# gvtulder/elasticdeform

Measured on AMD Instinct MI355X. Metric: Mvoxels/s fwd+grad, 256^3 fp32 order=3, higher is better.
Workload: dtype f32; 1 GPU; cfg2: 3D 256x256x256 float32, 5x5x5 grid sigma 5, order 3, mode mirror, prefilter on, deform_grid + deform_grid_gradient per step, one volume per GPU; parallelism=1 volume per GPU, no collective

## Files before the change

elasticdeform_amd/csrc/deform_k1z.hip:

```cpp
#include <hip/hip_runtime.h>

#include <cstring>
#include <type_traits>

#include "ed_device.h"
#include "ed_gridfilter.h"
#include "ed_params.h"
#include "ed_tile.h"
#include "ed_workspace.h"
#include "ed_zwalk.h"

namespace ed {
namespace tile {

#ifdef EDHIP_K1_STATS
__device__ unsigned long long g_k1z_stats[8];
#define ZSTAT(K, N) atomicAdd(&g_k1z_stats[K], (unsigned long long)(N))
#else
#define ZSTAT(K, N) do { } while (0)
#endif

namespace {


// ... 2 lines not shown
    kZStaged = 2,
    kZFast = 4,
    kZDma = 8,
    kZXin = 16,
    kZZYin = 32,
    kZUnfit = 64,
    kZGen = 128,
};
struct ZRecU {
    int b0z, b0y, b0x, flags, pitch, ez, ey, ex, goff, plane;
};
typedef int zv8i __attribute__((ext_vector_type(8)));
typedef const __attribute__((address_space(4))) zv8i* crec_p;
__device__ __forceinline__ ZRecU zrec_unpack(const zv8i& v)
{
    ZRecU r;
    r.b0z = v[0];
    r.b0y = v[1];
    r.b0x = v[2];
    r.flags = v[3];
    r.pitch = (v[3] >> 8) & 255;
    r.ez = v[4] & 1023;
    r.ey = (v[4] >> 10) & 1023;
    r.ex = (int)((unsigned)v[4] >> 20);
    r.goff = v[5];
    r.plane = r.ey * r.pitch;
    return r;
}
__device__ __forceinline__ ZRecU zrec_load(crec_p p)
{
    const zv8i v = *p;
    return zrec_unpack(v);
}

__host__ __device__ __forceinline__ int zctl(int parity, int list, int xcd) { return (parity * 2 + list) * 8 + xcd; }

#define ED_RED6(CTRL)                                      \
    "v_min_i32_dpp %0, %0, %0 " CTRL "\n\t"                \
    "v_min_i32_dpp %1, %1, %1 " CTRL "\n\t"                \
    "v_min_i32_dpp %2, %2, %2 " CTRL "\n\t"                \
    "v_max_i32_dpp %3, %3, %3 " CTRL "\n\t"                \
    "v_max_i32_dpp %4, %4, %4 " CTRL "\n\t"                \
    "v_max_i32_dpp %5, %5, %5 " CTRL "\n\t"
__device__ __forceinline__ void zrow_box(int (&lo)[3], int (&hi)[3])
{
    asm volatile("s_nop 1\n\t"
                 ED_RED6("quad_perm:[1,0,3,2] row_mask:0xf bank_mask:0xf")
                 ED_RED6("quad_perm:[2,3,0,1] row_mask:0xf bank_mask:0xf")
                 ED_RED6("row_half_mirror row_mask:0xf bank_mask:0xf")
                 ED_RED6("row_mirror row_mask:0xf bank_mask:0xf")
                 : "+v"(lo[0]), "+v"(lo[1]), "+v"(lo[2]), "+v"(hi[0]), "+v"(hi[1]), "+v"(hi[2]));
}
#undef ED_RED6
__device__ __forceinline__ int zuni(int v) { return __builtin_amdgcn_readfirstlane(v); }
__device__ __forceinline__ void zlds_barrier() { asm volatile("s_waitcnt lgkmcnt(0)\n\ts_barrier" ::: "memory"); }
__device__ __forceinline__ void zdma_barrier() { asm volatile("s_waitcnt vmcnt(0) lgkmcnt(0)\n\ts_barrier" ::: "memory"); }
__device__ __forceinline__ void zglds16(const float* g, float* lds)
{
    __builtin_amdgcn_global_load_lds((const __attribute__((address_space(1))) void*)g,
                                     (__attribute__((address_space(3))) void*)lds, 16, 0, 0);
}
template <bool OUT16>
__device__ __forceinline__ void zstore_out(float* img, long long off, float val, int io16)
{
    if constexpr (OUT16)
        reinterpret_cast<unsigned short*>(img)[off] = (unsigned short)narrow16(val, io16);
    else
        __builtin_nontemporal_store(val, img + off);
}

__device__ __forceinline__ void zaxis_entry(const GridGeom& g, int a, int oi, double* w, int* idx)
{
    const double cp = control_coordinate(g.ncp[a], (int64_t)oi + g.off[a], g.in_len[a]);
    const int64_t start = window_start(cp, 3);
    const bool edge = start < 0 || start + 3 >= g.ncp[a];
    spline_weights(cp, 3, w);
#pragma unroll
    for (int l = 0; l < 4; ++l)
        idx[l] = edge ? mirror_i32((int)start + l, (int)g.ncp[a]) : (int)start + l;
}

constexpr int kGeoBlock = 256;
constexpr int kGeoWaves = kGeoBlock / 64;
__global__ __launch_bounds__(kGeoBlock) void k1z_geo_kernel(const GridGeom g, const HotGeom hg, const ZGeom zg,
                                                          const GridPrefilter gp)
{
    extern __shared__ __attribute__((aligned(16))) char smem[];
    const int tid = threadIdx.x;
    const int lane = tid & 63;
    const int wave = zuni(tid >> 6);
    const int sample = blockIdx.y;
    const int ncpz = (int)g.ncp[0], ncpy = (int)g.ncp[1], ncpx = (int)g.ncp[2];
    const int nyx = ncpy * ncpx;
    const int ngrid = 3 * ncpz * nyx;
    double* sG = reinterpret_cast<double*>(smem);
    double* sR = sG + ngrid;
    AxTab* sAx = reinterpret_cast<AxTab*>(sR + 64 * ncpz * 3);
    double* sMax = reinterpret_cast<double*>(sAx + 16);
    AxTab* sZ = reinterpret_cast<AxTab*>(sMax + 3 * kGeoWaves);
    int* sCls = reinterpret_cast<int*>(sZ + 4 * hg.tiles[0]);
    int* sBox = sCls + hg.tiles[0];
    int* sCnt = sBox + 64 * hg.tiles[0];
    if ((int)blockIdx.x >= hg.tiles[1] * hg.tiles[2]) {
        const long long nfill = (long long)(gridDim.x - hg.tiles[1] * hg.tiles[2]) * kGeoBlock;
        const long long me = (long long)(blockIdx.x - hg.tiles[1] * hg.tiles[2]) * kGeoBlock + tid;
        const long long n16 = zg.zero_bytes >> 4;
        int4* p16 = reinterpret_cast<int4*>(zg.zero_ptr);
        for (long long i = me; i < n16; i += nfill)
            p16[i] = make_int4(0, 0, 0, 0);
        if (me < (zg.zero_bytes & 15))
            zg.zero_ptr[(n16 << 4) + me] = 0;
        return;
    }
    const int ty = blockIdx.x / hg.tiles[2], tx = blockIdx.x - ty * hg.tiles[2];
    if (ED_DBG(hg.dbg, 1 << 23))
        return;
#ifdef EDHIP_EXPERIMENTS
#define ZTICK(K) do { if (hg.dbgbuf && tid == 0) hg.dbgbuf[(size_t)(blockIdx.x + blockIdx.y * gridDim.x) * 16 + (K)] = __builtin_readcyclecounter(); } while (0)
#else
#define ZTICK(K) do { } while (0)
#endif
    ZTICK(0);

    if (gp.total > 0 && !ED_DBG(hg.dbg, 1 << 28)) {
        grid_prefilter_in_lds<kGeoBlock>(gp, sG, tid);
        if (blockIdx.x == 0 && sample == 0)
            for (int e = tid; e < gp.total; e += kGeoBlock)
                store_cast(gp.out + (int64_t)e * gp.elem_size, gp.dtype, sG[e]);
    } else {
        const char* disp = g.disp + (int64_t)sample * zg.disp_bstride;
        for (int e = tid; e < ngrid; e += kGeoBlock) {
            const int h = e / (ncpz * nyx), r = e - h * (ncpz * nyx);
            const int j0 = r / nyx, j = r - j0 * nyx;
            const int j1 = j / ncpx, j2 = j - j1 * ncpx;
            sG[e] = load_as_double(disp + g.disp_stride[0] * h + g.disp_stride[1] * j0 + g.disp_stride[2] * j1 +
                                       g.disp_stride[3] * j2, g.disp_dtype);
        }
        __syncthreads();
    }
    ZTICK(1);
    if (blockIdx.x == 0 && sample == 0 && tid == 0 && zg.hint) {
        if (zg.hint_host)
            __hip_atomic_store(zg.hint_host, ((unsigned long long)(unsigned)zg.hint[1] << 32) | (unsigned)zg.hint[0],
                               __ATOMIC_RELAXED, __HIP_MEMORY_SCOPE_SYSTEM);
        zg.hint[0] = 0;
        zg.hint[1] = (int)zg.hint_seq;
    }
    for (int h = 0; h < 3 && !ED_DBG(hg.dbg, 1 << 29); ++h) {
        double m = 0.0;
        for (int e = tid; e < ncpz * nyx; e += kGeoBlock)
            m = fmax(m, fabs(sG[h * ncpz * nyx + e]));
        for (int sh = 32; sh >= 1; sh >>= 1)
            m = fmax(m, __shfl_xor(m, sh));
        if (lane == 0)
            sMax[h * kGeoWaves + wave] = m;
    }
    ZTICK(2);
    if (tid < 16 && !ED_DBG(hg.dbg, 1 << 30)) {
        const int a = tid < 8 ? 1 : 2;
        const int oi = min((tid < 8 ? ty : tx) * kT + (tid & 7), hg.out_len[a] - 1);
        AxTab t;
        zaxis_entry(g, a, oi, t.w, t.idx);
        sAx[tid] = t;
    }
    for (int e = tid; e < 4 * hg.tiles[0] && !zg.tables_only && !ED_DBG(hg.dbg, 1 << 26); e += kGeoBlock) {
        const int tz = e >> 2, nz = min(kT, hg.out_len[0] - tz * kT);
        AxTab t;
        zaxis_entry(g, 0, tz * kT + ((e & 3) * (nz - 1)) / 3, t.w, t.idx);
        sZ[e] = t;
    }
    if (blockIdx.x == 0 && sample == 0 && hg.nstep) {
        for (long long ss = tid; ss < hg.nsteps; ss += kGeoBlock) {
            long long vol_off = 0, img_off = 0, r = ss;
            for (int l = 0; l < hg.nstep; ++l) {
                const long long q = r / hg.step_len[l];
                const long long c = r - q * hg.step_len[l];
                vol_off += hg.vol_step[l] * c;
                img_off += hg.img_step[l] * c;
                r = q;
            }
            zg.steps[2 * ss] = vol_off;
            zg.steps[2 * ss + 1] = img_off;
        }
    }
    if (blockIdx.x == 0 && sample == 0 && tid == 0) {
        ZGen* zn = reinterpret_cast<ZGen*>(zg.zgen);
        for (int h = 0; h < 3; ++h) {
            zn->in_len[h] = hg.in_len[h];
            zn->out_len[h] = hg.out_len[h];
            zn->off[h] = hg.off[h];
            zn->period[h] = hg.period[h];
            zn->inv_period[h] = hg.inv_period[h];
            zn->offd[h] = (double)hg.off[h];
        }
        for (int k = 0; k < 12; ++k)
            zn->aff[k] = hg.affine[k];
        zn->mode = hg.mode;
        zn->cval = hg.cval;
        zn->hint = hg.hint;
    }
    if (blockIdx.x == 0 && sample == 0) {
        AxTab* zt = const_cast<AxTab*>(zg.zt);
        for (int oz = tid; oz < hg.out_len[0]; oz += kGeoBlock) {
            AxTab t;
            zaxis_entry(g, 0, oz, t.w, t.idx);
#pragma unroll
            for (int l = 0; l < 4; ++l)
                t.idx[l] *= 32;
            zt[oz] = t;
        }
    }
    __syncthreads();
    ZTICK(3);
    double slack[3];
#pragma unroll
    for (int h = 0; h < 3; ++h) {
        double m = 0.0;
        for (int w = 0; w < kGeoWaves; ++w)
            m = fmax(m, sMax[h * kGeoWaves + w]);
        const double sl = zg.slack_scale * m;
        slack[h] = sl >= 0.02 ? (sl <= 0.75 ? sl : 0.75) : 0.02;
    }
    ZTICK(4);
    if (!ED_DBG(hg.dbg, 1 << 25)) {
        const int col = tid & 63;
        const AxTab ay = sAx[col >> 3];
        const AxTab ax = sAx[8 + (col & 7)];
        int rowoff[4];
#pragma unroll
        for (int ly = 0; ly < 4; ++ly)
            rowoff[ly] = ay.idx[ly] * ncpx;
        for (int r = tid >> 6; r < ncpz * 3; r += kGeoWaves) {
            const int kz = r / 3, h = r - kz * 3;
            const double* gp0 = sG + (h * ncpz + kz) * nyx;
            double acc = 0.0;
#pragma unroll
            for (int ly = 0; ly < 4; ++ly) {
                const double* row = gp0 + rowoff[ly];
                double t = ax.w[0] * row[ax.idx[0]];
#pragma unroll
                for (int lx = 1; lx < 4; ++lx)
                    t = fma(ax.w[lx], row[ax.idx[lx]], t);
                acc = fma(ay.w[ly], t, acc);
            }
            sR[col * (ncpz * 3) + r] = acc;
        }
        __syncthreads();
        double* rg = const_cast<double*>(zg.r) + (int64_t)sample * zg.r_bstride;
        const int rowlen = 8 * 4 * ncpz;
        for (int e = tid; e < 8 * rowlen; e += kGeoBlock) {
            const int py = e / rowlen, j = e - py * rowlen;
            const int px = j / (4 * ncpz), jj = j - px * (4 * ncpz);
            const int kz = jj >> 2, h = jj & 3;
            const int oy = ty * kT + py, ox = tx * kT + px;
            if (oy < hg.out_len[1] && ox < hg.out_len[2])
                rg[((int64_t)oy * hg.out_len[2] + ox) * (4 * ncpz) + jj] = h < 3 ? sR[(py * 8 + px) * (ncpz * 3) + kz * 3 + h] : 0.0;
        }
    }
    if (zg.tables_only)
        return;
    __syncthreads();
    ZTICK(5);
    const int order = zg.order;
    const int H = order / 2, NT = order + 1, kPadX = NT & 1;
    const int ny = min(kT, hg.out_len[1] - ty * kT), nx = min(kT, hg.out_len[2] - tx * kT);
    const int py = (((lane >> 2) & 3) * (ny - 1)) / 3, px = ((lane & 3) * (nx - 1)) / 3;
    const double* rc = sR + (py * 8 + px) * (ncpz * 3);
    for (int tz = wave; tz < hg.tiles[0] && !ED_DBG(hg.dbg, 1 << 24); tz += kGeoWaves) {
        const int nz = min(kT, hg.out_len[0] - tz * kT);
        const int pz = ((lane >> 4) * (nz - 1)) / 3;
        const int o[3] = {tz * kT + pz, ty * kT + py, tx * kT + px};
        const AxTab& ze = sZ[tz * 4 + (lane >> 4)];
        double d[3];
#pragma unroll
        for (int h = 0; h < 3; ++h) {
            d[h] = ze.w[0] * rc[ze.idx[0] * 3 + h];
#pragma unroll
            for (int l = 1; l < 4; ++l)
                d[h] = fma(ze.w[l], rc[ze.idx[l] * 3 + h], d[h]);
        }
        double c[3];
        int lo[3], hi[3];
#pragma unroll
        for (int h = 0; h < 3; ++h) {
            if (hg.has_affine)
                c[h] = fma(hg.affine[h * 4 + 2], (double)o[2],
                           fma(hg.affine[h * 4 + 0], (double)o[0],
                               fma(hg.affine[h * 4 + 1], (double)o[1], hg.affine[h * 4 + 3] + (double)hg.off[h]))) + d[h];
            else
                c[h] = (double)(o[h] + hg.off[h]) + d[h];
            const double cr = (order & 1) ? c[h] : c[h] + 0.5;
            lo[h] = (int)floor(cr - slack[h]);
            hi[h] = (int)floor(cr + slack[h]);
        }
        bool out_of_fast = false;
#pragma unroll
        for (int h = 0; h < 3; ++h)
            out_of_fast = out_of_fast || lo[h] < ((order & 1) ? 0 : 1) || hi[h] > hg.in_len[h] - 2;
        const bool fast = nz == kT && ny == kT && nx == kT && !__any(out_of_fast);
        zrow_box(lo, hi);
        int* dst = sBox + (tz * 8 + (lane >> 4)) * 8;
        if ((lane & 15) == 0) {
#pragma unroll
            for (int h = 0; h < 3; ++h) {
                dst[h] = lo[h];
                dst[4 + h] = hi[h];
            }
        }
        if (lane == 0)
            dst[3] = fast ? 1 : 0;
        if (!fast) {
            bool cst = false;
#pragma unroll
            for (int h = 0; h < 3; ++h) {
                double m = c[h];
                if (!(m >= 0.0 && m <= (double)(hg.in_len[h] - 1)))
                    m = map_coordinate_fast(m, hg.in_len[h], hg.mode, hg.period[h], hg.inv_period[h]);
                cst = cst || !(m > -1.0);
                const double mr = (order & 1) ? m : m + 0.5;
                lo[h] = (int)floor(mr - slack[h]);
                hi[h] = (int)floor(mr + slack[h]);
            }
            if (cst) {
#pragma unroll
                for (int h = 0; h < 3; ++h) {
                    lo[h] = 0x7fffffff;
                    hi[h] = (int)0x80000000;
                }
            }
            zrow_box(lo, hi);
            if ((lane & 15) == 0) {
#pragma unroll
                for (int h = 0; h < 3; ++h) {
                    dst[32 + h] = lo[h];
                    dst[36 + h] = hi[h];
                }
            }
        }
    }
    __syncthreads();
    ZTICK(6);
    for (int tz = tid; tz < hg.tiles[0] && !ED_DBG(hg.dbg, 1 << 27); tz += kGeoBlock) {
        const int tile_id = sample * hg.ntiles + (tz * hg.tiles[1] + ty) * hg.tiles[2] + tx;
        int cls = 0;
        bool hint0 = false, half_fit[2] = {false, false};
#pragma unroll 1
        for (int part = 0; part < 3; ++part) {
            const int* sb = sBox + tz * 64;
            const bool fast = sb[3] != 0;
            const int r0 = part == 2 ? 2 : 0, r1 = part == 1 ? 2 : 3;
            int blo[3], bhi[3];
            bool any = true;
#pragma unroll
            for (int h = 0; h < 3; ++h) {
                int rlo = 0x7fffffff, rhi = (int)0x80000000, lo = 0x7fffffff, hi = (int)0x80000000;
                for (int r = r0; r <= r1; ++r) {
                    rlo = min(rlo, sb[r * 8 + h]);
                    rhi = max(rhi, sb[r * 8 + 4 + h]);
                    lo = min(lo, sb[(fast ? 0 : 32) + r * 8 + h]);
                    hi = max(hi, sb[(fast ? 0 : 32) + r * 8 + 4 + h]);
                }
                if (!fast) {
                    any = any && hi >= lo;
                    const int lowfold = hg.mode == EDHIP_MODE_REFLECT ? -1 : 0;
                    if (rlo < ((order & 1) ? 0 : 1) && rhi >= lowfold)
                        lo = min(lo, lowfold);
                    if (rhi > hg.in_len[h] - 2 && rlo <= hg.in_len[h] - 1)
                        hi = max(hi, hg.in_len[h] - 1);
                }
                blo[h] = lo - H;
                bhi[h] = hi - H + order + (h == 2 ? kPadX : 0);
            }
            if (!any) {
                blo[0] = blo[1] = blo[2] = 0;
                bhi[0] = bhi[1] = bhi[2] = -1;
            }
            any = bhi[0] >= blo[0] && bhi[1] >= blo[1] && bhi[2] >= blo[2];
            unsigned ext[3];
#pragma unroll
            for (int h = 0; h < 3; ++h)
                ext[h] = (unsigned)bhi[h] - (unsigned)blo[h] + 1u;
            const int pitch = ext[2] <= 16u ? 16 : (ext[2] <= 24u ? 24 : (ext[2] <= 32u ? 32 : (ext[2] <= 48u ? 48 : 0)));
            const bool sane = any && ext[0] < 1024u && ext[1] < 1024u;
            const int nrows = sane ? (int)(ext[0] * ext[1]) : 0;
            const bool fits = sane && pitch > 0 && nrows * pitch <= hg.box_cap;
            const bool dma = fits && blo[2] >= 0 && blo[2] + pitch + 1 <= hg.in_len[2];
            const bool xin = fits && blo[2] >= 0 && blo[2] + (int)ext[2] <= hg.in_len[2];
            const bool zyin = fits && blo[0] >= 0 && blo[0] + (int)ext[0] <= hg.in_len[0] && blo[1] >= 0 &&
                              blo[1] + (int)ext[1] <= hg.in_len[1];
            const bool fastA = part == 0 && fast && fits && dma && zyin;
            const int flags = (any ? kZAny : 0) | (fits ? kZStaged : 0) | (fastA ? kZFast : kZGen) | (dma ? kZDma : 0) |
                              (xin ? kZXin : 0) | (zyin ? kZZYin : 0) | (any && !fits ? kZUnfit : 0);
            const int4 w0 = make_int4(blo[0], blo[1], blo[2], flags | (pitch << 8));
            const int4 w1 = make_int4(sane ? (int)(ext[0] | (ext[1] << 10) | (ext[2] << 20)) : 0,
                                      (dma && zyin) ? blo[0] * hg.vol_sz + blo[1] * hg.vol_sy + blo[2] : 0, 0, 0);
            if (part == 0) {
                hint0 = any && !(sane && pitch > 0 && nrows * pitch <= hg.small_cap);
                cls = (flags & kZUnfit) ? 3 : ((flags & kZFast) ? 1 : 2);
                int4* dst = reinterpret_cast<int4*>(zg.recs + (size_t)tile_id * 8);
                dst[0] = w0;
                dst[1] = w1;
                if (hg.boxes) {
                    int* bx = hg.boxes + (size_t)tile_id * 8;
#pragma unroll
                    for (int h = 0; h < 3; ++h) {
                        bx[h] = blo[h];
                        bx[3 + h] = bhi[h] - ((h == 2 && any) ? kPadX : 0);
                    }
                }
                if (cls != 3)
                    break;
            } else {
                half_fit[part - 1] = fits || !any;
                int4* dst = reinterpret_cast<int4*>(zg.recs_half + ((size_t)tile_id * 2 + (part - 1)) * 8);
                dst[0] = w0;
                dst[1] = w1;
            }
        }
        const bool split = cls == 3 && half_fit[0] && half_fit[1];
        ZSTAT(cls == 3 ? (split ? 6 : 5) : (cls == 1 ? 3 : 4), 1);
        sCls[tz] = cls | (split ? 4 : 0) | (hint0 ? 8 : 0);
    }
    __syncthreads();
    ZTICK(7);
    {
        const int zstrips = (hg.tiles[0] + zg.strip_tiles - 1) / zg.strip_tiles;
        if (tid < 4)
            sCnt[tid] = 0;
        __syncthreads();
        int slotG = -1, slotF = -1, sidv = 0;
        if (tid < zstrips) {
            int info = 0;
            bool g = false, f = false;
            for (int k = 0; k < zg.strip_tiles && tid * zg.strip_tiles + k < hg.tiles[0]; ++k) {
                const int c = sCls[tid * zg.strip_tiles + k];
                info |= c << (4 * k);
                g = g || (c & 3) == 2 || (c & 7) == 7;
                f = f || (c & 7) == 3;
            }
            const size_t sid = (size_t)sample * zg.nstrips + ((size_t)tid * hg.tiles[1] + ty) * hg.tiles[2] + tx;
            sidv = (int)sid;
            zg.sinfo[sid] = info;
            zg.missed[sid] = f ? 2 : 0;
            if (g)
                slotG = atomicAdd(&sCnt[0], 1);
            if (f)
                slotF = atomicAdd(&sCnt[1], 1);
        }
        __syncthreads();
        const int xcd = (tx + ty + sample) & 7;
        if (tid == 0) {
            sCnt[2] = sCnt[0] ? atomicAdd(&zg.ctl[zctl(zg.parity, 0, xcd)], sCnt[0]) : 0;
            sCnt[3] = sCnt[1] ? atomicAdd(&zg.ctl[zctl(zg.parity, 1, xcd)], sCnt[1]) : 0;
        }
        if (blockIdx.x == 0 && sample == 0 && tid < 16)
            zg.ctl[zctl(1 - zg.parity, tid >> 3, tid & 7)] = 0;
        __syncthreads();
        if (slotG >= 0)
            zg.list_g[(size_t)(sCnt[2] + slotG) * 8 + xcd] = sidv;
        if (slotF >= 0)
            zg.list_f[(size_t)(sCnt[3] + slotF) * 8 + xcd] = sidv;
    }
    ZTICK(8);
#undef ZTICK
}


struct ZVox {
    int addr[2];
    float frac[2][3];
    int flg;
};
struct ZStrip {
    int tz0, ty, tx, ntile, sample, id;
};
__device__ __forceinline__ bool k1z_strip(int total_strips, int nstrips, int tiles_z, int tiles_y, int tiles_x, int strip_tiles, int deal,
                                          ZStrip& sp, int b)
{
    const int x = b & 7, j = b >> 3;
    const int r = j / deal;
    int s = (r * 8 + ((x + r) & 7)) * deal + (j - r * deal);
    if (s >= total_strips)
        return false;
    sp.id = s;
    sp.sample = s / nstrips;
    s -= sp.sample * nstrips;
    sp.tx = s % tiles_x;
    s /= tiles_x;
    sp.ty = s % tiles_y;
    sp.tz0 = (s / tiles_y) * strip_tiles;
    sp.ntile = min(strip_tiles, tiles_z - sp.tz0);
    return true;
}
inline unsigned k1z_grid(int total_strips, int deal)
{
    const int chunks = (total_strips + deal - 1) / deal;
    return (unsigned)(((chunks + 7) / 8) * 8 * deal);
}

template <int ORDER, int PITCH>
__device__ __forceinline__ float k1z_gather(const float* bp, int plane, int pitch_rt, const float* w0, const float* w1, const float* w2)
{
    constexpr int NT = ORDER + 1;
    constexpr int NTX = NT + (NT & 1);
    float a0 = 0.f;
#pragma unroll
    for (int l0 = 0; l0 < NT; ++l0) {
        const float* pp = bp + l0 * plane;
        float a1 = 0.f;
#pragma unroll
        for (int l1 = 0; l1 < NT; ++l1) {
            const float* rp = pp + l1 * (PITCH ? PITCH : pitch_rt);
            float a2 = 0.f;
#pragma unroll
            for (int l2 = 0; l2 < NTX; l2 += 2) {
                const float2 pr = *reinterpret_cast<const float2*>(rp + l2);
                ED_NO_DS_MERGE();
                a2 = fmaf(w2[l2], pr.x, a2);
                a2 = fmaf(w2[l2 + 1], pr.y, a2);
            }
            a1 = fmaf(w1[l1], a2, a1);
        }
        a0 = fmaf(w0[l0], a1, a0);
    }
    return a0;
}
template <int ORDER>
__device__ __forceinline__ float k1z_voxel(const char* smem, int addr, const float (&frac)[3], int pitch, int plane)
{
    constexpr int NT = ORDER + 1;
    constexpr int NTX = NT + (NT & 1);
    float f0 = frac[0], f1 = frac[1], f2 = frac[2];
    asm volatile("" : "+v"(f0), "+v"(f1), "+v"(f2));
    float w0[NT], w1[NT], w2[NTX];
    weights_from_frac<float, ORDER>(f0, w0);
    weights_from_frac<float, ORDER>(f1, w1);
    weights_from_frac<float, ORDER>(f2, w2);
    if (NT & 1)
        w2[NT] = 0.f;
    const float* bp = reinterpret_cast<const float*>(smem + addr);
// ... 520 lines not shown
                    }
                    const long long ooff = (long long)oz * img_sz + obase;
                    ZSTAT(whole ? 2 : 1, 1);
                    for (int ss = 0; ss < nsteps; ++ss) {
                        float val = zn->cval;
                        if (!cst) {
                            const float* src = vol + (STEPS ? steps[2 * ss] : 0);
                            float a0 = 0.f;
#pragma unroll
                            for (int l0 = 0; l0 < NT; ++l0) {
                                float a1 = 0.f;
#pragma unroll
                                for (int l1 = 0; l1 < NT; ++l1) {
                                    const float* p1 = src + (tap[0][l0] + tap[1][l1]);
                                    float a2 = 0.f;
#pragma unroll
                                    for (int l2 = 0; l2 < NT; ++l2)
                                        a2 = fmaf(w[2][l2], p1[tap[2][l2]], a2);
                                    a1 = fmaf(w[1][l1], a2, a1);
                                }
                                a0 = fmaf(w[0][l0], a1, a0);
                            }
                            val = a0;
                        }
                        zstore_out<OUT16>(img, (STEPS ? steps[2 * ss + 1] : 0) + ooff, val, io16);
                    }
                }
            }
        }
    }
}

template <int ORDER, bool AFFINE, bool OUT16, bool STEPS>
hipError_t launch_k1z_kernels(const ZFast& zf, const void* znp, unsigned ngen, unsigned nfix, size_t lds, hipStream_t stream, SideLane*)
{
    const unsigned nfast = k1z_grid(zf.total_strips, zf.deal);
    const unsigned fast_rows = nfast >> 3, gen_rows = ngen >> 3;
    unsigned every = gen_rows ? fast_rows / gen_rows + 1 : 2;
    if (every < 2)
        every = 2;
    hipLaunchKernelGGL((k1z_tile_kernel<ORDER, AFFINE, OUT16, STEPS>), dim3(nfast + ngen), dim3(kBlock), lds, stream, zf, (czgen_p)znp,
                       (int)ngen, (int)every);
    hipError_t e = hipGetLastError();
    if (e != hipSuccess)
        return e;
    hipLaunchKernelGGL((k1z_fix_kernel<ORDER, AFFINE, OUT16, STEPS>), dim3(nfix, 2 * zf.strip_tiles), dim3(kBlock), 0, stream, zf, (czgen_p)znp);
    return hipGetLastError();
}
template <int ORDER, bool AFFINE, bool OUT16>
hipError_t launch_k1z_variant(const ZFast& zf, const void* zn, unsigned ngen, unsigned nfix, size_t lds, hipStream_t stream, SideLane* side,
                              bool steps)
{
    return steps ? launch_k1z_kernels<ORDER, AFFINE, OUT16, true>(zf, zn, ngen, nfix, lds, stream, side)
                 : launch_k1z_kernels<ORDER, AFFINE, OUT16, false>(zf, zn, ngen, nfix, lds, stream, side);
}
template <int ORDER>
hipError_t launch_k1z_order(const HotGeom& hg, const ZFast& zf, const void* zn, unsigned ngen, unsigned nfix, size_t lds, hipStream_t stream,
                            SideLane* side)
{
    const bool steps = hg.nstep != 0;
    if (hg.io16)
        return hg.has_affine ? launch_k1z_variant<ORDER, true, true>(zf, zn, ngen, nfix, lds, stream, side, steps)
                             : launch_k1z_variant<ORDER, false, true>(zf, zn, ngen, nfix, lds, stream, side, steps);
    return hg.has_affine ? launch_k1z_variant<ORDER, true, false>(zf, zn, ngen, nfix, lds, stream, side, steps)
                         : launch_k1z_variant<ORDER, false, false>(zf, zn, ngen, nfix, lds, stream, side, steps);
}

}

size_t k1z_lds_bytes(int* box_cap, bool large)
{
    size_t budget = large ? 52 * 1024 : 31 * 1024;
    if (const char* kb = ed_env("EDHIP_ZKB"))
        budget = (size_t)atoi(kb) * 1024;
    size_t cap = budget / 8;
    cap = ((cap - 56) / 64) * 64 + 56;
    *box_cap = (int)cap;
    return 2 * 4 * cap;
}

size_t k1z_geo_lds_bytes(const GridGeom& g, const HotGeom& hg)
{
    const size_t ngrid = 3 * (size_t)g.ncp[0] * (size_t)g.ncp[1] * (size_t)g.ncp[2];
    return 8 * ngrid + 8 * 64 * 3 * (size_t)g.ncp[0] + 16 * sizeof(AxTab) + 3 * kGeoWaves * 8 + (sizeof(AxTab) * 4 + 4 + 256) * (size_t)hg.tiles[0] + 16;
}

size_t k1z_r_bytes(const GridGeom& g) { return 8 * (size_t)g.out_len[1] * (size_t)g.out_len[2] * 4 * (size_t)g.ncp[0]; }

bool k1z_supported(const GridGeom& g)
{
    const size_t ngrid = 3 * (size_t)g.ncp[0] * (size_t)g.ncp[1] * (size_t)g.ncp[2];
    const size_t tiles_z = (size_t)((g.out_len[0] + kT - 1) / kT);
    return ngrid <= 4096 && g.ncp[0] <= 16 &&
           8 * ngrid + 8 * 64 * 3 * (size_t)g.ncp[0] + 16 * sizeof(AxTab) + 3 * kGeoWaves * 8 + (sizeof(AxTab) * 4 + 4 + 256) * tiles_z + 16 <= 60 * 1024;
}

hipError_t launch_k1z_geo(const GridGeom& g, const HotGeom& hg, const ZGeom& zg, const GridPrefilter& gp, int nbatch,
                          hipStream_t stream)
{
    unsigned fill = 0;
    if (zg.zero_ptr && zg.zero_bytes > 0) {
        const long long want = (zg.zero_bytes + 65535) / 65536;
        fill = (unsigned)(want < 1 ? 1 : (want > 2048 ? 2048 : want));
    }
    hipLaunchKernelGGL(k1z_geo_kernel, dim3((unsigned)(hg.tiles[1] * hg.tiles[2]) + fill, (unsigned)nbatch), dim3(kGeoBlock),
                       k1z_geo_lds_bytes(g, hg), stream, g, hg, zg, gp);
    if (ed_env("EDHIP_GEO_TWICE"))
        hipLaunchKernelGGL(k1z_geo_kernel, dim3((unsigned)(hg.tiles[1] * hg.tiles[2]) + fill, (unsigned)nbatch), dim3(kGeoBlock),
                           k1z_geo_lds_bytes(g, hg), stream, g, hg, zg, gp);
    return hipGetLastError();
}

hipError_t launch_k1z(const HotGeom& hg, const ZGeom& zg, int order, size_t lds, hipStream_t stream, SideLane* side)
{
    ZFast zf;
    memset(&zf, 0, sizeof(zf));
    zf.vol = hg.vol_r;
    zf.img = hg.img_w;
    zf.r = zg.r;
    zf.zt = zg.zt;
    zf.recs = zg.recs;
    zf.recs_half = zg.recs_half;
    zf.missed = zg.missed;
    zf.hint = hg.hint;
    zf.sinfo = zg.sinfo;
    zf.list_g = zg.list_g;
    zf.list_f = zg.list_f;
    zf.ctl = zg.ctl;
    zf.parity = zg.parity;
    zf.steps = zg.steps;
    zf.vol_bstride = hg.vol_bstride;
    zf.img_bstride = hg.img_bstride;
    zf.r_bstride = zg.r_bstride;
    zf.vol_sy = hg.vol_sy;
    zf.vol_sz = hg.vol_sz;
    zf.img_sy = hg.img_sy;
    zf.img_sz = hg.img_sz;
    zf.box_cap = hg.box_cap;
    zf.tiles_z = hg.tiles[0];
    zf.tiles_y = hg.tiles[1];
    zf.tiles_x = hg.tiles[2];
    zf.strip_tiles = zg.strip_tiles;
    zf.nstrips = zg.nstrips;
    zf.total_strips = zg.total_strips;
    zf.ntiles = hg.ntiles;
    zf.rcol_bytes = 32 * zg.ncpz;
    zf.out_y = hg.out_len[1];
    zf.out_x = hg.out_len[2];
    const int H = order / 2;
    zf.kz0 = (hg.has_affine ? 0 : hg.off[0]) - H;
    zf.ky0 = (hg.has_affine ? 0 : hg.off[1]) - H;
    zf.kx0 = (hg.has_affine ? 0 : hg.off[2]) - H;
    zf.io16 = hg.io16;
    zf.nsteps = (int)hg.nsteps;
    zf.dbg = hg.dbg;
    zf.deal = 4 * hg.tiles[2];
    while (zf.deal > 1 && zg.total_strips < 16 * zf.deal)
        zf.deal >>= 1;
    if (const char* dl = ed_env("EDHIP_ZDEAL"))
        zf.deal = atoi(dl) >= 1 ? atoi(dl) : zf.deal;
    for (int h = 0; h < 3; ++h) {
        for (int k = 0; k < 3; ++k)
            zf.aff[h * 4 + k] = hg.affine[h * 4 + k];
        zf.aff[h * 4 + 3] = hg.affine[h * 4 + 3] + (double)hg.off[h];
    }
    const void* zn = zg.zgen;
    unsigned ngen = (unsigned)(zg.total_strips < 1280 ? ((zg.total_strips + 7) / 8) * 8 : 1280);
    if (const char* ng = ed_env("EDHIP_ZNGEN"))
        ngen = (unsigned)((atoi(ng) + 7) / 8 * 8);
    const unsigned nfix = (unsigned)(zg.total_strips < 512 ? ((zg.total_strips + 7) / 8) * 8 : 512);
    switch (order) {
    case 1: return launch_k1z_order<1>(hg, zf, zn, ngen, nfix, lds, stream, side);
    case 2: return launch_k1z_order<2>(hg, zf, zn, ngen, nfix, lds, stream, side);
    case 3: return launch_k1z_order<3>(hg, zf, zn, ngen, nfix, lds, stream, side);
    default: return hipErrorNotSupported;
    }
}

#ifdef EDHIP_K1_STATS
extern "C" int edhip_debug_k1z_stats(unsigned long long* out8)
{
    unsigned long long z[8] = {0, 0, 0, 0, 0, 0, 0, 0};
    if (hipMemcpyFromSymbol(out8, HIP_SYMBOL(g_k1z_stats), sizeof(z)) != hipSuccess)
        return 1;
    return hipMemcpyToSymbol(HIP_SYMBOL(g_k1z_stats), z, sizeof(z)) != hipSuccess;
}
#endif

}
}
```

elasticdeform_amd/csrc/ed_gridfilter.h:

```cpp
#pragma once
#include "ed_device.h"
#include "ed_params.h"

namespace ed {

template <int N>
__device__ __forceinline__ void grid_filter_line(double* c, int inner, double z, double gain, double zn1)
{
#pragma clang fp contract(off)
    double v[N];
#pragma unroll
    for (int i = 0; i < N; ++i)
        v[i] = c[i * inner] * gain;
    double c0 = v[0] + zn1 * v[N - 1];
    double zi = z;
#pragma unroll
    for (int i = 1; i < N - 1; ++i) {
        c0 += zi * (v[i] + zn1 * v[N - 1 - i]);
        zi *= z;
    }
    c0 /= 1 - zn1 * zn1;
    v[0] = c0;
#pragma unroll
    for (int i = 1; i < N; ++i)
        v[i] += z * v[i - 1];
    v[N - 1] = (z * v[N - 2] + v[N - 1]) * z / (z * z - 1);
#pragma unroll
    for (int i = N - 2; i >= 0; --i)
        v[i] = z * (v[i + 1] - v[i]);
#pragma unroll
    for (int i = 0; i < N; ++i)
        c[i * inner] = v[i];
}

template <int NT>
__device__ __forceinline__ void grid_prefilter_in_lds(const GridPrefilter& p, double* s, int tid)
{
#pragma clang fp contract(off)
    const int total = p.total;
    for (int e = tid; e < total; e += NT) {
        int r = e;
        int64_t off = 0;
        for (int d = p.ndim - 1; d >= 0; --d) {
            const int q = r / p.shape[d];
            off += (int64_t)(r - q * p.shape[d]) * p.stride_bytes[d];
            r = q;
        }
        s[e] = load_as_double(p.in + off, p.dtype);
    }
    __syncthreads();
    const double z = p.pole, gain = p.gain;
    for (int ax = 1; ax < p.ndim; ++ax) {
        const int n = p.shape[ax];
        int inner = 1;
        for (int d = ax + 1; d < p.ndim; ++d)
            inner *= p.shape[d];
        const int nlines = total / n;
        if (n >= 2) {
            const double zn1 = p.pole_pow[ax];
            for (int line = tid; line < nlines; line += NT) {
                const int outer = line / inner, in = line - outer * inner;
                double* c = s + (int64_t)outer * n * inner + in;
                switch (n) {
                case 2: grid_filter_line<2>(c, inner, z, gain, zn1); continue;
                case 3: grid_filter_line<3>(c, inner, z, gain, zn1); continue;
                case 4: grid_filter_line<4>(c, inner, z, gain, zn1); continue;
                case 5: grid_filter_line<5>(c, inner, z, gain, zn1); continue;
                case 6: grid_filter_line<6>(c, inner, z, gain, zn1); continue;
                case 7: grid_filter_line<7>(c, inner, z, gain, zn1); continue;
                case 8: grid_filter_line<8>(c, inner, z, gain, zn1); continue;
                default: break;
                }
                for (int i = 0; i < n; ++i)
                    c[i * inner] *= gain;
                double c0 = c[0] + zn1 * c[(n - 1) * inner];
                double zi = z;
                for (int i = 1; i < n - 1; ++i) {
                    c0 += zi * (c[i * inner] + zn1 * c[(n - 1 - i) * inner]);
                    zi *= z;
                }
                c0 /= 1 - zn1 * zn1;
                c[0] = c0;
                for (int i = 1; i < n; ++i)
                    c[i * inner] += z * c[(i - 1) * inner];
                c[(n - 1) * inner] = (z * c[(n - 2) * inner] + c[(n - 1) * inner]) * z / (z * z - 1);
                for (int i = n - 2; i >= 0; --i)
                    c[i * inner] = z * (c[(i + 1) * inner] - c[i * inner]);
            }
        }
        __syncthreads();
        if (p.dtype != EDHIP_F64) {
            for (int e = tid; e < total; e += NT) {
                char tmp[8];
                store_cast(tmp, p.dtype, s[e]);
                s[e] = load_as_double(tmp, p.dtype);
            }
            __syncthreads();
        }
    }
}

}
```

Measured before the change: 25980 Mvoxels/s.

## Split k1z geo duties into dedicated block and cut barriers in setup

Moves the one-off duties (hint publish, step table, ZGen header, z table, ctl reset, prefilter output store) from block 0 into an extra dedicated block so patch blocks no longer wait on them. Patch blocks now compute per-component max with one wave each, assign the axis-table and z-table work to separate waves, and use a lighter zlds_barrier in place of several __syncthreads. It adds a separable x-then-y pass through a new LDS scratch buffer that is used only when it fits, and rewrites the R store loop row-wise with a float reciprocal for the index split. The grid prefilter now rounds to storage dtype inside the line filter instead of in an extra full pass with barriers. This adds LDS use and an extra block, and the float-reciprocal index math could go wrong for large row lengths.

```diff
diff --git a/elasticdeform_amd/csrc/deform_k1z.hip b/elasticdeform_amd/csrc/deform_k1z.hip
--- a/elasticdeform_amd/csrc/deform_k1z.hip
+++ b/elasticdeform_amd/csrc/deform_k1z.hip
@@ -108,6 +108,15 @@
 
 constexpr int kGeoBlock = 256;
 constexpr int kGeoWaves = kGeoBlock / 64;
+__host__ __device__ inline size_t k1z_geo_base_bytes(size_t ngrid, size_t ncpz, size_t tiles_z)
+{
+    return 8 * ngrid + 8 * 64 * 3 * ncpz + 16 * sizeof(AxTab) + 3 * kGeoWaves * 8 + (sizeof(AxTab) * 4 + 4 + 256) * tiles_z + 16;
+}
+__host__ __device__ inline size_t k1z_geo_t_bytes(size_t ngrid, size_t ncpx, size_t ncpz, size_t tiles_z)
+{
+    const size_t rows = ngrid / ncpx;
+    return rows <= 128 && k1z_geo_base_bytes(ngrid, ncpz, tiles_z) + 64 * rows + 8 <= 60 * 1024 ? 64 * rows + 8 : 0;
+}
 __global__ __launch_bounds__(kGeoBlock) void k1z_geo_kernel(const GridGeom g, const HotGeom hg, const ZGeom zg,
                                                           const GridPrefilter gp)
 {
@@ -127,9 +136,10 @@
     int* sCls = reinterpret_cast<int*>(sZ + 4 * hg.tiles[0]);
     int* sBox = sCls + hg.tiles[0];
     int* sCnt = sBox + 64 * hg.tiles[0];
-    if ((int)blockIdx.x >= hg.tiles[1] * hg.tiles[2]) {
-        const long long nfill = (long long)(gridDim.x - hg.tiles[1] * hg.tiles[2]) * kGeoBlock;
-        const long long me = (long long)(blockIdx.x - hg.tiles[1] * hg.tiles[2]) * kGeoBlock + tid;
+    const int npatch = hg.tiles[1] * hg.tiles[2];
+    if ((int)blockIdx.x > npatch) {
+        const long long nfill = (long long)(gridDim.x - npatch - 1) * kGeoBlock;
+        const long long me = (long long)(blockIdx.x - npatch - 1) * kGeoBlock + tid;
         const long long n16 = zg.zero_bytes >> 4;
         int4* p16 = reinterpret_cast<int4*>(zg.zero_ptr);
         for (long long i = me; i < n16; i += nfill)
@@ -138,6 +148,9 @@
             zg.zero_ptr[(n16 << 4) + me] = 0;
         return;
     }
+    const bool duties = (int)blockIdx.x == npatch;
+    if (duties && sample != 0)
+        return;
     const int ty = blockIdx.x / hg.tiles[2], tx = blockIdx.x - ty * hg.tiles[2];
     if (ED_DBG(hg.dbg, 1 << 23))
         return;
@@ -148,11 +161,67 @@
 #endif
     ZTICK(0);
 
+    if (duties) {
+        if (tid == 0 && zg.hint) {
+            if (zg.hint_host)
+                __hip_atomic_store(zg.hint_host, ((unsigned long long)(unsigned)zg.hint[1] << 32) | (unsigned)zg.hint[0],
+                                   __ATOMIC_RELAXED, __HIP_MEMORY_SCOPE_SYSTEM);
+            zg.hint[0] = 0;
+            zg.hint[1] = (int)zg.hint_seq;
+        }
+        if (hg.nstep) {
+            for (long long ss = tid; ss < hg.nsteps; ss += kGeoBlock) {
+                long long vol_off = 0, img_off = 0, r = ss;
+                for (int l = 0; l < hg.nstep; ++l) {
+                    const long long q = r / hg.step_len[l];
+                    const long long c = r - q * hg.step_len[l];
+                    vol_off += hg.vol_step[l] * c;
+                    img_off += hg.img_step[l] * c;
+                    r = q;
+                }
+                zg.steps[2 * ss] = vol_off;
+                zg.steps[2 * ss + 1] = img_off;
+            }
+        }
+        if (tid == kGeoBlock - 1) {
+            ZGen* zn = reinterpret_cast<ZGen*>(zg.zgen);
+            for (int h = 0; h < 3; ++h) {
+                zn->in_len[h] = hg.in_len[h];
+                zn->out_len[h] = hg.out_len[h];
+                zn->off[h] = hg.off[h];
+                zn->period[h] = hg.period[h];
+                zn->inv_period[h] = hg.inv_period[h];
+                zn->offd[h] = (double)hg.off[h];
+            }
+            for (int k = 0; k < 12; ++k)
+                zn->aff[k] = hg.affine[k];
+            zn->mode = hg.mode;
+            zn->cval = hg.cval;
+            zn->hint = hg.hint;
+        }
+        {
+            AxTab* zt = const_cast<AxTab*>(zg.zt);
+            for (int oz = tid; oz < hg.out_len[0]; oz += kGeoBlock) {
+                AxTab t;
+                zaxis_entry(g, 0, oz, t.w, t.idx);
+#pragma unroll
+                for (int l = 0; l < 4; ++l)
+                    t.idx[l] *= 32;
+                zt[oz] = t;
+            }
+        }
+        if (!zg.tables_only && tid < 16)
+            zg.ctl[zctl(1 - zg.parity, tid >> 3, tid & 7)] = 0;
+        if (gp.total > 0 && !ED_DBG(hg.dbg, 1 << 28)) {
+            grid_prefilter_in_lds<kGeoBlock>(gp, sG, tid);
+            for (int e = tid; e < gp.total; e += kGeoBlock)
+                store_cast(gp.out + (int64_t)e * gp.elem_size, gp.dtype, sG[e]);
+        }
+        return;
+    }
+
     if (gp.total > 0 && !ED_DBG(hg.dbg, 1 << 28)) {
         grid_prefilter_in_lds<kGeoBlock>(gp, sG, tid);
-        if (blockIdx.x == 0 && sample == 0)
-            for (int e = tid; e < gp.total; e += kGeoBlock)
-                store_cast(gp.out + (int64_t)e * gp.elem_size, gp.dtype, sG[e]);
     } else {
         const char* disp = g.disp + (int64_t)sample * zg.disp_bstride;
         for (int e = tid; e < ngrid; e += kGeoBlock) {
@@ -165,127 +234,112 @@
         __syncthreads();
     }
     ZTICK(1);
-    if (blockIdx.x == 0 && sample == 0 && tid == 0 && zg.hint) {
-        if (zg.hint_host)
-            __hip_atomic_store(zg.hint_host, ((unsigned long long)(unsigned)zg.hint[1] << 32) | (unsigned)zg.hint[0],
-                               __ATOMIC_RELAXED, __HIP_MEMORY_SCOPE_SYSTEM);
-        zg.hint[0] = 0;
-        zg.hint[1] = (int)zg.hint_seq;
-    }
-    for (int h = 0; h < 3 && !ED_DBG(hg.dbg, 1 << 29); ++h) {
+    if (wave < 3 && !ED_DBG(hg.dbg, 1 << 29)) {
+        const int h = wave;
         double m = 0.0;
-        for (int e = tid; e < ncpz * nyx; e += kGeoBlock)
+        for (int e = lane; e < ncpz * nyx; e += 64)
             m = fmax(m, fabs(sG[h * ncpz * nyx + e]));
         for (int sh = 32; sh >= 1; sh >>= 1)
             m = fmax(m, __shfl_xor(m, sh));
         if (lane == 0)
-            sMax[h * kGeoWaves + wave] = m;
-    }
-    ZTICK(2);
-    if (tid < 16 && !ED_DBG(hg.dbg, 1 << 30)) {
-        const int a = tid < 8 ? 1 : 2;
-        const int oi = min((tid < 8 ? ty : tx) * kT + (tid & 7), hg.out_len[a] - 1);
+            sMax[h] = m;
+    }
+    if (wave == kGeoWaves - 1 && lane < 16 && !ED_DBG(hg.dbg, 1 << 30)) {
+        const int a = lane < 8 ? 1 : 2;
+        const int oi = min((lane < 8 ? ty : tx) * kT + (lane & 7), hg.out_len[a] - 1);
         AxTab t;
         zaxis_entry(g, a, oi, t.w, t.idx);
-        sAx[tid] = t;
-    }
-    for (int e = tid; e < 4 * hg.tiles[0] && !zg.tables_only && !ED_DBG(hg.dbg, 1 << 26); e += kGeoBlock) {
+        sAx[lane] = t;
+    }
+    for (int e = tid ^ (kGeoBlock - 64); e < 4 * hg.tiles[0] && !zg.tables_only && !ED_DBG(hg.dbg, 1 << 26); e += kGeoBlock) {
         const int tz = e >> 2, nz = min(kT, hg.out_len[0] - tz * kT);
         AxTab t;
         zaxis_entry(g, 0, tz * kT + ((e & 3) * (nz - 1)) / 3, t.w, t.idx);
         sZ[e] = t;
     }
-    if (blockIdx.x == 0 && sample == 0 && hg.nstep) {
-        for (long long ss = tid; ss < hg.nsteps; ss += kGeoBlock) {
-            long long vol_off = 0, img_off = 0, r = ss;
-            for (int l = 0; l < hg.nstep; ++l) {
-                const long long q = r / hg.step_len[l];
-                const long long c = r - q * hg.step_len[l];
-                vol_off += hg.vol_step[l] * c;
-                img_off += hg.img_step[l] * c;
-                r = q;
-            }
-            zg.steps[2 * ss] = vol_off;
-            zg.steps[2 * ss + 1] = img_off;
-        }
-    }
-    if (blockIdx.x == 0 && sample == 0 && tid == 0) {
-        ZGen* zn = reinterpret_cast<ZGen*>(zg.zgen);
-        for (int h = 0; h < 3; ++h) {
-            zn->in_len[h] = hg.in_len[h];
-            zn->out_len[h] = hg.out_len[h];
-            zn->off[h] = hg.off[h];
-            zn->period[h] = hg.period[h];
-            zn->inv_period[h] = hg.inv_period[h];
-            zn->offd[h] = (double)hg.off[h];
-        }
-        for (int k = 0; k < 12; ++k)
-            zn->aff[k] = hg.affine[k];
-        zn->mode = hg.mode;
-        zn->cval = hg.cval;
-        zn->hint = hg.hint;
-    }
-    if (blockIdx.x == 0 && sample == 0) {
-        AxTab* zt = const_cast<AxTab*>(zg.zt);
-        for (int oz = tid; oz < hg.out_len[0]; oz += kGeoBlock) {
-            AxTab t;
-            zaxis_entry(g, 0, oz, t.w, t.idx);
-#pragma unroll
-            for (int l = 0; l < 4; ++l)
-                t.idx[l] *= 32;
-            zt[oz] = t;
-        }
-    }
-    __syncthreads();
+    zlds_barrier();
+    ZTICK(2);
+    double slack[3];
+#pragma unroll
+    for (int h = 0; h < 3; ++h) {
+        const double sl = zg.slack_scale * fmax(0.0, sMax[h]);
+        slack[h] = sl >= 0.02 ? (sl <= 0.75 ? sl : 0.75) : 0.02;
+    }
     ZTICK(3);
-    double slack[3];
-#pragma unroll
-    for (int h = 0; h < 3; ++h) {
-        double m = 0.0;
-        for (int w = 0; w < kGeoWaves; ++w)
-            m = fmax(m, sMax[h * kGeoWaves + w]);
-        const double sl = zg.slack_scale * m;
-        slack[h] = sl >= 0.02 ? (sl <= 0.75 ? sl : 0.75) : 0.02;
-    }
-    ZTICK(4);
     if (!ED_DBG(hg.dbg, 1 << 25)) {
         const int col = tid & 63;
         const AxTab ay = sAx[col >> 3];
-        const AxTab ax = sAx[8 + (col & 7)];
-        int rowoff[4];
-#pragma unroll
-        for (int ly = 0; ly < 4; ++ly)
-            rowoff[ly] = ay.idx[ly] * ncpx;
-        for (int r = tid >> 6; r < ncpz * 3; r += kGeoWaves) {
-            const int kz = r / 3, h = r - kz * 3;
-            const double* gp0 = sG + (h * ncpz + kz) * nyx;
-            double acc = 0.0;
-#pragma unroll
-            for (int ly = 0; ly < 4; ++ly) {
-                const double* row = gp0 + rowoff[ly];
-                double t = ax.w[0] * row[ax.idx[0]];
-#pragma unroll
-                for (int lx = 1; lx < 4; ++lx)
-                    t = fma(ax.w[lx], row[ax.idx[lx]], t);
-                acc = fma(ay.w[ly], t, acc);
-            }
-            sR[col * (ncpz * 3) + r] = acc;
-        }
-        __syncthreads();
+        const size_t t_bytes = k1z_geo_t_bytes((size_t)ngrid, (size_t)ncpx, (size_t)ncpz, (size_t)hg.tiles[0]);
+        if (t_bytes) {
+            double* sT = reinterpret_cast<double*>(smem + (((reinterpret_cast<char*>(sCnt + 4) - smem) + 7) & ~7));
+            const int nrow = 3 * ncpz * ncpy;
+            {
+                const AxTab ax = sAx[8 + (tid & 7)];
+                for (int row_i = tid >> 3; row_i < nrow; row_i += kGeoBlock / 8) {
+                    const double* row = sG + row_i * ncpx;
+                    double t = ax.w[0] * row[ax.idx[0]];
+#pragma unroll
+                    for (int lx = 1; lx < 4; ++lx)
+                        t = fma(ax.w[lx], row[ax.idx[lx]], t);
+                    sT[row_i * 8 + (tid & 7)] = t;
+                }
+            }
+            zlds_barrier();
+            int rowoff[4];
+#pragma unroll
+            for (int ly = 0; ly < 4; ++ly)
+                rowoff[ly] = ay.idx[ly] * 8 + (col & 7);
+            for (int r = tid >> 6; r < ncpz * 3; r += kGeoWaves) {
+                const int kz = r / 3, h = r - kz * 3;
+                const double* tp0 = sT + (h * ncpz + kz) * (ncpy * 8);
+                double acc = 0.0;
+#pragma unroll
+                for (int ly = 0; ly < 4; ++ly)
+                    acc = fma(ay.w[ly], tp0[rowoff[ly]], acc);
+                sR[col * (ncpz * 3) + r] = acc;
+            }
+        } else {
+            const AxTab ax = sAx[8 + (col & 7)];
+            int rowoff[4];
+#pragma unroll
+            for (int ly = 0; ly < 4; ++ly)
+                rowoff[ly] = ay.idx[ly] * ncpx;
+            for (int r = tid >> 6; r < ncpz * 3; r += kGeoWaves) {
+                const int kz = r / 3, h = r - kz * 3;
+                const double* gp0 = sG + (h * ncpz + kz) * nyx;
+                double acc = 0.0;
+#pragma unroll
+                for (int ly = 0; ly < 4; ++ly) {
+                    const double* row = gp0 + rowoff[ly];
+                    double t = ax.w[0] * row[ax.idx[0]];
+#pragma unroll
+                    for (int lx = 1; lx < 4; ++lx)
+                        t = fma(ax.w[lx], row[ax.idx[lx]], t);
+                    acc = fma(ay.w[ly], t, acc);
+                }
+                sR[col * (ncpz * 3) + r] = acc;
+            }
+        }
+        zlds_barrier();
+        ZTICK(4);
         double* rg = const_cast<double*>(zg.r) + (int64_t)sample * zg.r_bstride;
-        const int rowlen = 8 * 4 * ncpz;
-        for (int e = tid; e < 8 * rowlen; e += kGeoBlock) {
-            const int py = e / rowlen, j = e - py * rowlen;
-            const int px = j / (4 * ncpz), jj = j - px * (4 * ncpz);
-            const int kz = jj >> 2, h = jj & 3;
-            const int oy = ty * kT + py, ox = tx * kT + px;
-            if (oy < hg.out_len[1] && ox < hg.out_len[2])
-                rg[((int64_t)oy * hg.out_len[2] + ox) * (4 * ncpz) + jj] = h < 3 ? sR[(py * 8 + px) * (ncpz * 3) + kz * 3 + h] : 0.0;
+        const int collen = 4 * ncpz, rowlen = 8 * collen;
+        const float inv_collen = __frcp_rn((float)collen);
+        for (int py = wave; py < 8; py += kGeoWaves) {
+            const int oy = ty * kT + py;
+            if (oy >= hg.out_len[1])
+                break;
+            double* rrow = rg + ((int64_t)oy * hg.out_len[2] + tx * kT) * collen;
+            for (int j = lane; j < rowlen; j += 64) {
+                const int px = (int)(((float)j + 0.5f) * inv_collen), jj = j - px * collen;
+                const int kz = jj >> 2, h = jj & 3;
+                if (tx * kT + px < hg.out_len[2])
+                    rrow[j] = h < 3 ? sR[(py * 8 + px) * (ncpz * 3) + kz * 3 + h] : 0.0;
+            }
         }
     }
     if (zg.tables_only)
         return;
-    __syncthreads();
     ZTICK(5);
     const int order = zg.order;
     const int H = order / 2, NT = order + 1, kPadX = NT & 1;
@@ -364,9 +418,11 @@
             }
         }
     }
-    __syncthreads();
+    if (tid < 4)
+        sCnt[tid] = 0;
+    zlds_barrier();
     ZTICK(6);
-    for (int tz = tid; tz < hg.tiles[0] && !ED_DBG(hg.dbg, 1 << 27); tz += kGeoBlock) {
+    for (int tz = lane * kGeoWaves + wave; tz < hg.tiles[0] && !ED_DBG(hg.dbg, 1 << 27); tz += kGeoBlock) {
         const int tile_id = sample * hg.ntiles + (tz * hg.tiles[1] + ty) * hg.tiles[2] + tx;
         int cls = 0;
         bool hint0 = false, half_fit[2] = {false, false};
@@ -447,13 +503,10 @@
         ZSTAT(cls == 3 ? (split ? 6 : 5) : (cls == 1 ? 3 : 4), 1);
         sCls[tz] = cls | (split ? 4 : 0) | (hint0 ? 8 : 0);
     }
-    __syncthreads();
+    zlds_barrier();
     ZTICK(7);
     {
         const int zstrips = (hg.tiles[0] + zg.strip_tiles - 1) / zg.strip_tiles;
-        if (tid < 4)
-            sCnt[tid] = 0;
-        __syncthreads();
         int slotG = -1, slotF = -1, sidv = 0;
         if (tid < zstrips) {
             int info = 0;
@@ -473,15 +526,13 @@
             if (f)
                 slotF = atomicAdd(&sCnt[1], 1);
         }
-        __syncthreads();
+        zlds_barrier();
         const int xcd = (tx + ty + sample) & 7;
         if (tid == 0) {
             sCnt[2] = sCnt[0] ? atomicAdd(&zg.ctl[zctl(zg.parity, 0, xcd)], sCnt[0]) : 0;
             sCnt[3] = sCnt[1] ? atomicAdd(&zg.ctl[zctl(zg.parity, 1, xcd)], sCnt[1]) : 0;
         }
-        if (blockIdx.x == 0 && sample == 0 && tid < 16)
-            zg.ctl[zctl(1 - zg.parity, tid >> 3, tid & 7)] = 0;
-        __syncthreads();
+        zlds_barrier();
         if (slotG >= 0)
             zg.list_g[(size_t)(sCnt[2] + slotG) * 8 + xcd] = sidv;
         if (slotF >= 0)
@@ -1168,7 +1219,8 @@
 size_t k1z_geo_lds_bytes(const GridGeom& g, const HotGeom& hg)
 {
     const size_t ngrid = 3 * (size_t)g.ncp[0] * (size_t)g.ncp[1] * (size_t)g.ncp[2];
-    return 8 * ngrid + 8 * 64 * 3 * (size_t)g.ncp[0] + 16 * sizeof(AxTab) + 3 * kGeoWaves * 8 + (sizeof(AxTab) * 4 + 4 + 256) * (size_t)hg.tiles[0] + 16;
+    return k1z_geo_base_bytes(ngrid, (size_t)g.ncp[0], (size_t)hg.tiles[0]) +
+           k1z_geo_t_bytes(ngrid, (size_t)g.ncp[2], (size_t)g.ncp[0], (size_t)hg.tiles[0]);
 }
 
 size_t k1z_r_bytes(const GridGeom& g) { return 8 * (size_t)g.out_len[1] * (size_t)g.out_len[2] * 4 * (size_t)g.ncp[0]; }
@@ -1177,8 +1229,7 @@
 {
     const size_t ngrid = 3 * (size_t)g.ncp[0] * (size_t)g.ncp[1] * (size_t)g.ncp[2];
     const size_t tiles_z = (size_t)((g.out_len[0] + kT - 1) / kT);
-    return ngrid <= 4096 && g.ncp[0] <= 16 &&
-           8 * ngrid + 8 * 64 * 3 * (size_t)g.ncp[0] + 16 * sizeof(AxTab) + 3 * kGeoWaves * 8 + (sizeof(AxTab) * 4 + 4 + 256) * tiles_z + 16 <= 60 * 1024;
+    return ngrid <= 4096 && g.ncp[0] <= 16 && k1z_geo_base_bytes(ngrid, (size_t)g.ncp[0], tiles_z) <= 60 * 1024;
 }
 
 hipError_t launch_k1z_geo(const GridGeom& g, const HotGeom& hg, const ZGeom& zg, const GridPrefilter& gp, int nbatch,
@@ -1189,10 +1240,10 @@
         const long long want = (zg.zero_bytes + 65535) / 65536;
         fill = (unsigned)(want < 1 ? 1 : (want > 2048 ? 2048 : want));
     }
-    hipLaunchKernelGGL(k1z_geo_kernel, dim3((unsigned)(hg.tiles[1] * hg.tiles[2]) + fill, (unsigned)nbatch), dim3(kGeoBlock),
+    hipLaunchKernelGGL(k1z_geo_kernel, dim3((unsigned)(hg.tiles[1] * hg.tiles[2]) + 1 + fill, (unsigned)nbatch), dim3(kGeoBlock),
                        k1z_geo_lds_bytes(g, hg), stream, g, hg, zg, gp);
     if (ed_env("EDHIP_GEO_TWICE"))
-        hipLaunchKernelGGL(k1z_geo_kernel, dim3((unsigned)(hg.tiles[1] * hg.tiles[2]) + fill, (unsigned)nbatch), dim3(kGeoBlock),
+        hipLaunchKernelGGL(k1z_geo_kernel, dim3((unsigned)(hg.tiles[1] * hg.tiles[2]) + 1 + fill, (unsigned)nbatch), dim3(kGeoBlock),
                            k1z_geo_lds_bytes(g, hg), stream, g, hg, zg, gp);
     return hipGetLastError();
 }
diff --git a/elasticdeform_amd/csrc/ed_gridfilter.h b/elasticdeform_amd/csrc/ed_gridfilter.h
--- a/elasticdeform_amd/csrc/ed_gridfilter.h
+++ b/elasticdeform_amd/csrc/ed_gridfilter.h
@@ -4,8 +4,27 @@
 
 namespace ed {
 
+__device__ __forceinline__ double grid_storage_round(double v, int dtype)
+{
+    switch (dtype) {
+    case EDHIP_F16: return (double)(float)(_Float16)(float)v;
+    case EDHIP_BF16: return (double)bf16_to_float(float_to_bf16((float)v));
+    case EDHIP_BOOL:
+    case EDHIP_U8: return (double)(uint8_t)trunc_i32(v);
+    case EDHIP_I8: return (double)(int8_t)trunc_i32(v);
+    case EDHIP_U16: return (double)(uint16_t)trunc_i32(v);
+    case EDHIP_I16: return (double)(int16_t)trunc_i32(v);
+    case EDHIP_U32: return (double)(uint32_t)trunc_i64(v);
+    case EDHIP_I32: return (double)trunc_i32(v);
+    case EDHIP_U64: return (double)trunc_u64(v);
+    case EDHIP_I64: return (double)trunc_i64(v);
+    case EDHIP_F32: return (double)(float)v;
+    default: return v;
+    }
+}
+
 template <int N>
-__device__ __forceinline__ void grid_filter_line(double* c, int inner, double z, double gain, double zn1)
+__device__ __forceinline__ void grid_filter_line(double* c, int inner, double z, double gain, double zn1, int dtype)
 {
 #pragma clang fp contract(off)
     double v[N];
@@ -30,7 +49,7 @@
         v[i] = z * (v[i + 1] - v[i]);
 #pragma unroll
     for (int i = 0; i < N; ++i)
-        c[i * inner] = v[i];
+        c[i * inner] = grid_storage_round(v[i], dtype);
 }
 
 template <int NT>
@@ -62,13 +81,13 @@
                 const int outer = line / inner, in = line - outer * inner;
                 double* c = s + (int64_t)outer * n * inner + in;
                 switch (n) {
-                case 2: grid_filter_line<2>(c, inner, z, gain, zn1); continue;
-                case 3: grid_filter_line<3>(c, inner, z, gain, zn1); continue;
-                case 4: grid_filter_line<4>(c, inner, z, gain, zn1); continue;
-                case 5: grid_filter_line<5>(c, inner, z, gain, zn1); continue;
-                case 6: grid_filter_line<6>(c, inner, z, gain, zn1); continue;
-                case 7: grid_filter_line<7>(c, inner, z, gain, zn1); continue;
-                case 8: grid_filter_line<8>(c, inner, z, gain, zn1); continue;
+                case 2: grid_filter_line<2>(c, inner, z, gain, zn1, p.dtype); continue;
+                case 3: grid_filter_line<3>(c, inner, z, gain, zn1, p.dtype); continue;
+                case 4: grid_filter_line<4>(c, inner, z, gain, zn1, p.dtype); continue;
+                case 5: grid_filter_line<5>(c, inner, z, gain, zn1, p.dtype); continue;
+                case 6: grid_filter_line<6>(c, inner, z, gain, zn1, p.dtype); continue;
+                case 7: grid_filter_line<7>(c, inner, z, gain, zn1, p.dtype); continue;
+                case 8: grid_filter_line<8>(c, inner, z, gain, zn1, p.dtype); continue;
                 default: break;
                 }
                 for (int i = 0; i < n; ++i)
@@ -86,17 +105,11 @@
                 c[(n - 1) * inner] = (z * c[(n - 2) * inner] + c[(n - 1) * inner]) * z / (z * z - 1);
                 for (int i = n - 2; i >= 0; --i)
                     c[i * inner] = z * (c[(i + 1) * inner] - c[i * inner]);
+                for (int i = 0; i < n; ++i)
+                    c[i * inner] = grid_storage_round(c[i * inner], p.dtype);
             }
         }
         __syncthreads();
-        if (p.dtype != EDHIP_F64) {
-            for (int e = tid; e < total; e += NT) {
-                char tmp[8];
-                store_cast(tmp, p.dtype, s[e]);
-                s[e] = load_as_double(tmp, p.dtype);
-            }
-            __syncthreads();
-        }
     }
 }
 
```

Result: no change. 25830 Mvoxels/s (-0.6%).
